# TinyMPC/tinympc-matlab

Hardware: AMD Instinct MI355X
Metric: ADMM iterations/s, batched quadrotor nx=12 nu=4 N=50 (instance-iterations/s, whole job) (higher is better)
Workload: dtype f64

## Files before the change

__graft_entry__.py:

```python
from __future__ import annotations

import hashlib
import importlib.util
import os
import shutil
import subprocess
import sys

ROOT = os.path.dirname(os.path.abspath(__file__))
if ROOT not in sys.path:
    sys.path.insert(0, ROOT)
PKG_DIR = os.path.join(ROOT, "tinympc-matlab_amd")
PKG_NAME = "tinympc_matlab_amd"
CSRC = os.path.join(PKG_DIR, "csrc")
HIP_LIB = os.path.join(PKG_DIR, "libtinympc_hip.so")
ORACLE_DIR = os.path.join(ROOT, "oracle")
REFERENCE_SRC = "/root/reference/src/codegen_src"

HIP_SOURCES = ["tinympc_kernels.hip", "tinympc_precompute_rows.hip", "tinympc_solve.hip", "tinympc_solve_b.hip", "tinympc_solve_fam.hip", "tinympc_solve_adapt.hip", "tinympc_solve_c.hip", "tinympc_solve_d.hip", "tinympc_solve_dr.hip", "tinympc_solve_dw.hip", "tinympc_solve_dx.hip", "tinympc_jit.hip", "tinympc_solve_m.hip", "tinympc_precompute_large.hip", "tinympc_handle.hip", "tinympc_plan.hip", "tinympc_session.hip", "tinympc_capi.hip",
               "tinympc_codegen.hip"]
HIP_LINTED = ["tinympc_precompute_rows.hip", "tinympc_solve.hip", "tinympc_solve_b.hip", "tinympc_solve_fam.hip", "tinympc_solve_adapt.hip",
              "tinympc_solve_c.hip", "tinympc_solve_d.hip", "tinympc_solve_dr.hip", "tinympc_solve_dw.hip", "tinympc_solve_dx.hip"]
JIT_EMBEDDED = ["tinympc_device.h", "tinympc_sweep.h", "tinympc_fam_red.h", "tinympc_solve_d_chain.h", "tinympc_solve_dw_chain.h", "tinympc_solve_dx_chain.h",
                "tinympc_solve_e_common.h", "tinympc_solve_dwide.h", "tinympc_solve_d.hip", "tinympc_solve_dw.hip", "tinympc_solve_dx.hip", "tinympc_solve_e.hip",
                "tinympc_solve_f.hip"]
_ROCKET = ["-DTINY_JIT_NX=6", "-DTINY_JIT_NU=3", "-DTINY_JIT_N=100", "-DTINY_JIT_CT=0", "-DTINY_JIT_FAM=1"]
_ROCKET_FAM = ["-DTINY_JIT_E_NROUND=1", "-DTINY_JIT_E_NCONE=2", "-DTINY_JIT_E_CONES={0,0,2},{0,6,8}", "-DTINY_JIT_E_NLX=1", "-DTINY_JIT_E_NLU=0"]
HIP_BUILTINS = [
    ("k_builtin_e_rocket100", "tinympc_solve_e.hip",
     _ROCKET + ["-DTINY_JIT_E_WPG=8", "-DTINY_JIT_E_WPS=2", "-DTINY_JIT_E_S=13"] + _ROCKET_FAM +
     ["-DTINY_JIT_E_GC_LDS=0", "-DTINY_JIT_E_GL_LDS=0", "-DTINY_JIT_E_LX_LDS=0", "-DTINY_JIT_E_KFAM=1", "-DTINY_JIT_E_DREG=1"]),
    ("k_builtin_f_rocket100", "tinympc_solve_f.hip", _ROCKET + ["-DTINY_JIT_F_WPG=4", "-DTINY_JIT_F_S=7"] + _ROCKET_FAM + ["-DTINY_JIT_F_KFAM=1"]),
    ("k_builtin_f_rocket100_session", "tinympc_solve_f.hip", _ROCKET + ["-DTINY_JIT_F_WPG=4", "-DTINY_JIT_F_S=7"] + _ROCKET_FAM + ["-DTINY_JIT_F_KFAM=1", "-DTINY_JIT_F_SESSION=1"]),
]
_NO_FAM = ["-DTINY_JIT_E_NROUND=0", "-DTINY_JIT_E_NCONE=0", "-DTINY_JIT_E_CONES={-1,0,0}", "-DTINY_JIT_E_NLX=0", "-DTINY_JIT_E_NLU=0"]
for _name, _nx, _nu, _N, _wpg, _S in (("cartpole20", 4, 1, 20, 2, 3), ("quadrotor50", 12, 4, 50, 4, 4)):
    for _suffix, _ct, _extra in (("", 1, []), ("_var", 0, []), ("_session", 0, ["-DTINY_JIT_F_SESSION=1"])):
        HIP_BUILTINS.append(("k_builtin_f_%s%s" % (_name, _suffix), "tinympc_solve_f.hip",
                             ["-DTINY_JIT_NX=%d" % _nx, "-DTINY_JIT_NU=%d" % _nu, "-DTINY_JIT_N=%d" % _N, "-DTINY_JIT_CT=%d" % _ct, "-DTINY_JIT_FAM=0",
                              "-DTINY_JIT_F_WPG=%d" % _wpg, "-DTINY_JIT_F_S=%d" % _S] + _NO_FAM + _extra))
BUILD_DIR = os.path.join(ROOT, "build", "hip")
HIP_CFLAGS = ["--offload-arch=gfx950", "-O3", "-std=c++17", "-fPIC", "-fno-gpu-rdc",
              "-Wall", "-Wno-unused-function", "-I" + os.path.join(ROOT, "include"), "-I" + CSRC, "-I" + BUILD_DIR]
HIP_LDFLAGS = ["--offload-arch=gfx950", "-shared", "-fPIC", "-fno-gpu-rdc", "-lhiprtc"]

# ... 296 lines not shown
```

tinympc-matlab_amd/csrc/tinympc_device.h:

```cpp
#pragma once
#ifndef __HIPCC_RTC__
#include <hip/hip_runtime.h>
#endif

namespace tinympc {

__host__ __device__ inline size_t ops_doubles(int W, int KT) { return (size_t)2 * W * KT + 3 * W; }

__host__ __device__ inline size_t table_rows(int N) { return (size_t)N + 2; }

constexpr int V_PAD = 4;
__host__ __device__ inline size_t v_rows(int N) { return (size_t)N + 1 + 2 * V_PAD; }
__host__ __device__ inline size_t tables_doubles(int W, int N) { return 3 * table_rows(N) * W + W; }

#if defined(__HIPCC__) || defined(__HIPCC_RTC__)
__device__ __forceinline__ void host_store(double *p, double v) { __hip_atomic_store(p, v, __ATOMIC_RELAXED, __HIP_MEMORY_SCOPE_SYSTEM); }
#endif

struct PrecomputeParams {
    int nx, nu;
    double rho;
    const double *A, *B, *fdyn, *Qd, *Rd;
    double *Kinf, *Pinf, *Quu_inv, *AmBKt, *APf, *BPf;
    int *info;
// ... 237 lines not shown
    double *rho_inst;
    int batch;
    double rho;
    double *mail;
};
hipError_t launch_setup_init(const SetupInitParams &p, hipStream_t stream);
hipError_t launch_fill_bounds(double *xmin, double *xmax, size_t X, double *umin, double *umax, size_t U, double inf, hipStream_t stream);
hipError_t launch_reset_stats(int *istats, double *dstats, double *rho_inst, int batch, double rho, hipStream_t stream);
size_t lqr_scratch_doubles(int nx, int nu);
size_t precompute_large_scratch_doubles(int nx, int nu);
hipError_t launch_precompute_large(const PrecomputeParams &p, hipStream_t stream);
hipError_t launch_build_operators(const OperatorParams &p, hipStream_t stream);
hipError_t launch_build_tables(const TableParams &p, hipStream_t stream);
hipError_t launch_store_inst_refs(const InstRefStoreParams &p, hipStream_t stream);
hipError_t launch_build_inst_tables(const InstTableParams &p, hipStream_t stream);
enum class SolveExt { Box, Families, Adaptive, InstRefs, InstBounds };
hipError_t launch_solve_a(const SolveParams &p, SolveExt ext, int W, int KT, size_t lds_bytes, hipStream_t stream);
hipError_t launch_solve_b(const SolveParams &p, int W, int KT, size_t lds_bytes, hipStream_t stream);
size_t solve_b_lds_bytes(int nx, int nu, int N, int W);
constexpr int WAVES_PER_GROUP_B = 4;
bool solve_d_supported(int nx, int nu, int N, bool const_tables);
hipError_t launch_solve_d(const SolveParams &p, hipStream_t stream);
hipError_t launch_solve_d_refill(const SolveParams &p, hipStream_t stream);
int solve_d_workgroups(int nu, int N, bool const_tables, int groups);
size_t solve_d_lds_bytes(int nu, int N, bool const_tables);
int solve_d_resident_workgroups(int wpg);
int solve_d_wavefronts_per_workgroup(int nu, int N, bool const_tables);
bool solve_dw_supported(int nx, int nu, int N, bool const_tables);
hipError_t launch_solve_dw(const SolveParams &p, hipStream_t stream);
int solve_dw_workgroups(int nu, int N, int groups);
size_t solve_dw_lds_bytes(int nu, int N);
bool solve_dx_supported(int nx, int nu, int N, bool const_tables);
hipError_t launch_solve_dx(const SolveParams &p, hipStream_t stream);
int solve_dx_workgroups(int nu, int N, int groups);
size_t solve_dx_lds_bytes(int nu, int N);
hipError_t launch_solve_c(const SolveParams &p, int W, int KT, size_t lds_bytes, hipStream_t stream);
hipError_t launch_build_chunk_tables(const ChunkTableParams &p, hipStream_t stream);
size_t f_input_table_doubles(int nu, int S);
hipError_t launch_build_f_input_tables(const ChunkTableParams &p, hipStream_t stream);
void chunk_plan(int N, int *S, int *C, int *Lc);
size_t solve_c_lds_bytes(int nx, int Lc);
size_t solve_c_lds_bytes_refs(int nx, int nu, int N, int Lc);
size_t chunk_table_doubles(int nx, int Lc);
int chunk_ks(int nx);
hipError_t launch_build_adapt(const AdaptTableParams &p, hipStream_t stream);
inline hipError_t ensure_dynamic_lds(const void *fn, size_t bytes, size_t (&cache)[16]) {
// ... 39 lines not shown
```

tinympc-matlab_amd/csrc/tinympc_plan.hip:

```cpp
#include <cstring>
#include "tinympc_handle.h"

using namespace tinympc;
using namespace tinympc::host;

namespace {

void arm_completion_flag(tinympc_solver *s, SolveParams &p) {
    if (!p.host_sol) return;
    s->session_seq += 1;
    p.host_seq = (double)s->session_seq;
    s->flag_pending = true;
}

void decide_layout_d_variants(tinympc_solver *s) {
    if (!s->layout_d) return;
    if (s->d_varying < 0 && !s->tables_const()) {
        if (s->W == 16 && !s->d_jit && solve_d_supported(s->nx, s->nu, s->N, false)) {
            s->d_varying = 1;
        } else {
            s->d_varying_jit = solve_jit_supported(s->W, s->nx, s->nu, s->N, false);
            s->d_varying = s->d_varying_jit ? 1 : 0;
        }
    }
// ... 185 lines not shown
}

static bool refill_applies(const tinympc_solver *s, const LaunchPlan &pl) {
    const bool jit = pl.kernel == KernelId::D_JIT;
    if ((pl.kernel != KernelId::D_COMPILED && !jit) || s->W != 16 || pl.adaptive || pl.families || pl.inst_refs || s->zero_copy_tick || s->st.max_iter <= 0 ||
        s->st.check_termination <= 0)
        return false;
    const char *env = getenv("TINYMPC_REFILL");
    const int mode = env ? atoi(env) : -1;
    if (mode == 0) return false;
    const bool ct = s->tables_const();
    long resident;
    if (jit) resident = solve_jit_resident_wavefronts(s->W, s->nx, s->nu, s->N, ct);
    else {
        const int wpg = solve_d_wavefronts_per_workgroup(s->nu, s->N, ct);
        resident = (long)solve_d_resident_workgroups(wpg) * wpg;
    }
    const bool reachable = s->st.abs_pri_tol > 0.0 && s->st.abs_dua_tol > 0.0;
    if ((long)s->groups <= resident) return false;
    if (!reachable && mode != 1) return false;
    return !jit || solve_jit_refill_supported(s->W, s->nx, s->nu, s->N, ct);
}

int launch(tinympc_solver *s, bool timed) {
    int rc;
    s->flag_pending = false;
    if ((rc = resolve_plan(s))) return rc;
    const LaunchPlan pl = current_plan(s);
    const bool fam = pl.families, adaptive = pl.adaptive;
    if (s->inst_tables() && !pl.inst_refs) {
        const bool r = s->inst.refs(), b = s->inst.bounds;
        return fail(TINYMPC_ERR_UNSUPPORTED, "%s%s%s are not supported %s; %s%s%s", r ? "per-instance references (set_x_ref_batch / set_u_ref_batch)" : "",
                    r && b ? " and " : "", b ? "per-instance bounds (set_bound_constraints_batch)" : "",
                    s->layout_m ? "for systems with nx+nu > 64" : fam ? "with cone / linear constraint families" : "with adaptive rho",
                    r ? "tinympc_set_x_ref / tinympc_set_u_ref return to shared references" : "", r && b ? ", " : "",
                    b ? "tinympc_set_bound_constraints returns to shared bounds" : "");
    }
    if (s->refs_on_host && adaptive) {
        if ((rc = flush_host_refs(s))) return rc;
    }
    if ((rc = refresh_derived(s))) return rc;
    if (adaptive && fam)
        return fail(TINYMPC_ERR_UNSUPPORTED, "adaptive_rho together with cone / linear constraint families is not supported");
    if (s->layout_m && adaptive)
        return fail(TINYMPC_ERR_UNSUPPORTED, "adaptive_rho is not supported for systems with nx+nu > 64");
    if (fam && pl.kernel != KernelId::E && pl.kernel != KernelId::F && pl.kernel != KernelId::M && family_structure(s).beyond_generic())
// ... 63 lines not shown
    }
    p.rho_min = s->st.adaptive_rho_min; p.rho_max = s->st.adaptive_rho_max; p.rho_clip = s->st.adaptive_rho_enable_clipping;
    const bool kernel_takes_cold = (pl.kernel == KernelId::D_COMPILED || pl.kernel == KernelId::D_JIT) && s->st.max_iter > 0;
    if (s->cold_state && !kernel_takes_cold && (rc = materialize_cold_state(s))) return rc;
    p.cold = s->cold_state ? 1 : 0;
    s->cold_state = false;
    if (s->st.max_iter > 0) s->sol_zero_pending = false;
    else if ((rc = materialize_zero_solution(s))) return rc;
    if (refill_applies(s, pl) && !p.x0_mirror && !p.u0_host && !p.host_sol) {
        if (!s->drefill && (rc = dalloc(s, &s->drefill, 1))) return rc;
        HIP_TRY(hipMemsetAsync(s->drefill, 0, sizeof(int), s->stream));
        p.refill_next = s->drefill;
    }
    if (timed) HIP_TRY(hipEventRecord(s->ev0, s->stream));
    switch (pl.kernel) {
        case KernelId::M:
            p.ctab = s->dctab;
            HIP_TRY(launch_solve_m(p, s->stream));
            break;
        case KernelId::D_JIT:
            HIP_TRY(launch_solve_jit(p, s->W, s->stream));
            break;
        case KernelId::D_COMPILED:
            HIP_TRY(s->W == 64 ? launch_solve_dx(p, s->stream) : s->W == 32 ? launch_solve_dw(p, s->stream) : launch_solve_d(p, s->stream));
            break;
        case KernelId::E:
            p.ctab = s->dctab_e; p.chunk_len = s->e_chunk_len; p.chunk_count = s->e_wpg; p.chunk_levels = 1;
            HIP_TRY(launch_solve_e(p, s->fs, s->stream));
            break;
        case KernelId::F:
            p.ctab = s->dctab_f; p.ftab = s->dftab; p.chunk_len = s->f_chunk_len; p.chunk_count = s->f_chunks; p.chunk_levels = 4;
            arm_completion_flag(s, p);
            HIP_TRY(launch_solve_f(p, s->f_fs, s->stream));
            break;
        case KernelId::C:
            p.ctab = s->dctab; p.chunk_len = s->chunk_len; p.chunk_count = s->chunk_count; p.chunk_levels = s->chunk_levels;
            arm_completion_flag(s, p);
            HIP_TRY(launch_solve_c(p, s->W, s->KT, s->lds_bytes_c, s->stream));
            break;
        case KernelId::B:
            HIP_TRY(launch_solve_b(p, s->W, s->KT, s->lds_bytes, s->stream));
            break;
        case KernelId::A:
        case KernelId::FAM_A:
        case KernelId::ADAPT_A: {
            const SolveExt ext = pl.kernel == KernelId::FAM_A ? SolveExt::Families : pl.kernel == KernelId::ADAPT_A ? SolveExt::Adaptive
                                 : pl.inst_bounds ? SolveExt::InstBounds : pl.inst_refs ? SolveExt::InstRefs : SolveExt::Box;
// ... 33 lines not shown
    if (rc) return rc;
    if ((rc = bind_device(s))) return rc;
    s->specialise_asked = true;
    if ((rc = resolve_plan(s))) return rc;
    (void)refill_applies(s, current_plan(s));
    return TINYMPC_OK;
}

int tinympc_get_jit_info(tinympc_solver *s, char *buf, int len) {
    int rc = check_handle(s);
    if (rc) return rc;
    if (!buf || len < 1) return fail(TINYMPC_ERR_INVALID_INPUT, "get_jit_info: buffer required");
    buf[0] = '\0';
    const LaunchPlan pl = current_plan(s);
    const bool ct = s->tables_const();
    if (pl.inst_refs) {
        const char *words = !pl.inst_bounds ? " per-instance-refs" : s->inst.refs() ? " per-instance-refs per-instance-bounds" : " per-instance-bounds";
        if (pl.kernel == KernelId::D_JIT) {
            if ((rc = bind_device(s))) return rc;
            solve_jit_describe(s->W, s->nx, s->nu, s->N, true, false, false, buf, (size_t)len, true);
            strncat(buf, words, (size_t)len - strlen(buf) - 1);
            strncat(buf, " goal", (size_t)len - strlen(buf) - 1);
        } else {
            snprintf(buf, (size_t)len, "compiled-in layout=%c%s%s", pl.layout, words, pl.kernel == KernelId::D_COMPILED ? " goal" : "");
        }
        return TINYMPC_OK;
    }
    if (!pl.adaptive && !s->f_sig.empty() && !s->f_ok && pl.kernel != KernelId::E && pl.kernel != KernelId::D_JIT && pl.kernel != KernelId::D_COMPILED)
        solve_f_describe(s->nx, s->nu, s->N, ct, pl.families, s->f_fs, buf, (size_t)len);
    else if (!pl.adaptive && !s->e_sig.empty() && !s->e_ok && pl.kernel != KernelId::F && pl.kernel != KernelId::D_JIT && pl.kernel != KernelId::D_COMPILED)
        solve_e_describe(s->nx, s->nu, s->N, ct, pl.families, s->fs, buf, (size_t)len);
    else if (pl.kernel == KernelId::F) solve_f_describe(s->nx, s->nu, s->N, ct, pl.families, s->f_fs, buf, (size_t)len);
    else if (pl.kernel == KernelId::E) solve_e_describe(s->nx, s->nu, s->N, ct, pl.families, s->fs, buf, (size_t)len);
    else if (pl.kernel == KernelId::D_JIT || (s->d_jit_asked && !s->layout_d && !s->layout_m)) {
        if ((rc = bind_device(s))) return rc;
        solve_jit_describe(s->W, s->nx, s->nu, s->N, ct, pl.families && !pl.adaptive, pl.adaptive && !pl.families, buf, (size_t)len);
        if (pl.kernel == KernelId::D_JIT && refill_applies(s, pl)) strncat(buf, " slot-refill", (size_t)len - strlen(buf) - 1);
    } else snprintf(buf, (size_t)len, "compiled-in layout=%c%s", pl.layout, refill_applies(s, pl) ? " slot-refill" : "");
    return TINYMPC_OK;
}

}
```

tinympc-matlab_amd/csrc/tinympc_solve_d.hip:

```cpp
#ifndef TINY_JIT
#include <atomic>
#endif
#include <type_traits>

#include "tinympc_device.h"
#include "tinympc_sweep.h"

#ifndef TINY_REFILL
#if defined(TINY_JIT_REFILL) && TINY_JIT_REFILL
#define TINY_REFILL 1
#else
#define TINY_REFILL 0
#endif
#endif

#define TINY_STR2(x) #x
#define TINY_STR(x) TINY_STR2(x)
namespace tinympc {
template <int NX, int NU>
struct DStep;
}

#ifdef TINY_JIT
#define D_NX TINY_JIT_NX
#define D_NU TINY_JIT_NU
#include "tinympc_solve_d_chain.h"
#else
#define D_NX 12
#define D_NU 4
#include "tinympc_solve_d_chain.h"
#define D_NX 4
#define D_NU 1
#include "tinympc_solve_d_chain.h"
#endif

namespace tinympc {
// ... 342 lines not shown
            static_for<0, 16>([&](auto K) {
                constexpr int o = (K.value < NXU ? K.value : 0) * 16;
                m[K.value] = fma(delta, src[o + (sAd - sOps)], src[o]);
            });
        } else {
            static_for<0, 16>([&](auto K) { m[K.value] = src[(K.value < NXU ? K.value : 0) * 16]; });
        }
    };
    auto vget = [&](auto S) -> double {
        if constexpr (decltype(S)::value >= VL) return Vr[decltype(S)::value - VL];
        else return sVl[decltype(S)::value * 64];
    };

#ifdef TINY_CLOCK_STAMP
    const unsigned long long ck_t0 = __builtin_amdgcn_s_memtime(), ck_r0 = __builtin_amdgcn_s_memrealtime();
#endif
#ifdef TINY_D_PAD
    asm volatile(".rept " TINY_STR(TINY_D_PAD) "\n\ts_nop 0\n\t.endr" ::: "memory");
#endif
#ifdef TINY_D_LOOP_ALIGN
    asm volatile(".p2align " TINY_STR(TINY_D_LOOP_ALIGN) ::: "memory");
#endif
    const int max_iter = p.max_iter;
    for (int it = 0; max_iter > 0; ++it) {
        const int it0 = __builtin_amdgcn_readfirstlane(it);
#if TINY_REFILL
        const bool final_round = REFILL ? false : it0 >= max_iter;
#else
        const bool final_round = it0 >= max_iter;
#endif
        if constexpr (TWO_PER_SIMD) fair_share_priority<NS>(it0, simd_slot);
#if TINY_REFILL
        const bool fin = REFILL ? it_done >= max_iter : final_round;
        const bool wb = pending || (fin && active);
#else
        const bool wb = pending || (final_round && active);
#endif
        if (TINY_RARE(__ballot(wb) != 0ull)) {
            int lane_o = lane;
            asm volatile("" : "+v"(lane_o));
            const int r_o = lane_o & 15, j_o = lane_o >> 4;
            const bool x_o = r_o < NX;
#if TINY_REFILL
            int cur_o = cur;
            if constexpr (REFILL) asm volatile("" : "+v"(cur_o));
            const size_t grp_w = REFILL ? (size_t)(cur_o >> 2) : (size_t)grp;
            const int lane_w = REFILL ? (cur_o & 3) * 16 + r_o : lane_o;
#endif
            if (wb && r_o < NXU) {
// ... 91 lines not shown
                        if (take) {
                            static_for<0, VL>([&](auto S) { sVl[S.value * 64] = 0.0; });
                            if (!x_o && r_o < NXU)
                                for (int i = 0; i < NS; ++i) sDw[i * DS] = 0.0;
                        }
                    } else if (take) {
                        const double *const nG = p.G + grp_n * (N + 1) * 64 + lane_n;
                        const double *const nV = p.V + (grp_n * v_rows(N) + V_PAD) * 64 + lane_n;
                        static_for<0, NS>([&](auto S) { G[S.value] = nG[(S.value + koff) * 64]; });
                        static_for<0, NVR>([&](auto S) { Vr[S.value] = nV[(VL + S.value + koff) * 64]; });
                        static_for<0, VL>([&](auto S) { sVl[S.value * 64] = nV[(S.value + koff) * 64]; });
                        G0 = nG[0];
                        V0 = nV[0];
                        if (!x_o && r_o < NXU) {
                            const double *const nD = p.D + grp_n * (NS * DS) + (nxt & 3) * NU + (r_o - NX);
                            for (int i = 0; i < NS; ++i) sDw[i * DS] = nD[i * DS];
                        }
                    }
#endif
                }
            }
            pending = false;
        }
        if (final_round || __ballot(active) == 0ull) break;
        const int it1 = it0 + 1;
#if TINY_REFILL
        bool chk = true, check_r = false;
        if constexpr (REFILL) {
            chk = active && (ct > 0) && (((it_done + 1) % ct) == 0);
            check_r = __ballot(chk) != 0ull;
        }
#define TINY_CHECK_PLAIN (__builtin_amdgcn_readfirstlane((int)((ct > 0) && ((it1 % ct) == 0))) != 0)
        const bool check = REFILL ? check_r : TINY_CHECK_PLAIN;
#undef TINY_CHECK_PLAIN
#else
        const bool check = __builtin_amdgcn_readfirstlane((int)((ct > 0) && ((it1 % ct) == 0))) != 0;
#endif

        double pri = 0.0, dua = 0.0;
        bool may = check;
        double m[16];
        load_ops(sMf, m);
        const bool adapt = ADAPT && __builtin_amdgcn_readfirstlane((int)((it0 > 0) && (it0 % 5 == 0))) != 0;
        double a_pr = 0.0, a_pn = 0.0, a_dr = 0.0, a_dn = 0.0;
        double gprev = 0.0;
        double mtr[16];
        if constexpr (ADAPT) {
            if (adapt) static_for<0, 16>([&](auto K) { mtr[K.value] = K.value < NXU ? sAd[2 * 256 + K.value * 16 + r] : 0.0; });
        }
// ... 9 lines not shown
#if TINY_REFILL
                may = __builtin_amdgcn_readfirstlane((int)wave_may_converge_d(__ballot(bad), __ballot(REFILL ? chk : active))) != 0;
#else
                may = __builtin_amdgcn_readfirstlane((int)wave_may_converge_d(__ballot(bad), __ballot(active))) != 0;
#endif
            }
#if TINY_REFILL
            if (TINY_RARE(may) && is_x && active) gV1u[REFILL ? row_offset(cur) : (unsigned)lane] = V0;
#else
            if (TINY_RARE(may) && is_x && active) gV1u[(unsigned)lane] = V0;
#endif
            V0 = snew;
        }
        if constexpr (FAM) {
            double gcn, gln;
            (void)families(x0v, GC0, GL0, gcn, gln);
            if (is_x) {
                GC0 = gcn;
                GL0 = gln;
            }
        }
        double xcur = x0v;
        double dcur = lds_read_async<0>(aD), vcur = 0.0;
        if constexpr (VL > 0) vcur = lds_read_async<0>(aV);
        double locur = lo_c, hicur = hi_c;
        if constexpr (!CT) {
            locur = lds_read_async<W * 8>(aT);
            hicur = lds_read_async<(TOFF + W) * 8>(aT);
        }
        lds_wait_ops(m);
        auto fstep = [&](auto S) {
            constexpr int q = decltype(S)::value;
            double dn = 0.0, vn = 0.0, lon = lo_c, hin = hi_c;
            if constexpr (q + 1 < NS) dn = lds_read_async<(q + 1) * DS * 8>(aD);
            if constexpr (q + 1 < VL) vn = lds_read_async<(q + 1) * 512>(aV);
            if constexpr (!CT && q + 1 < NS) {
                lon = lds_read_async<(q + 2) * W * 8>(aT);
                hin = lds_read_async<(TOFF + (q + 2) * W) * 8>(aT);
            }
            const double xprev = xcur;
            double snew_q;
            if constexpr (q >= VL) {
                if constexpr (K0 && q == 0) xcur = Step::fwd_reg0(dcur, m, c0, locur, hicur, G[q], Vr[q - VL], pri, dua);
                else xcur = Step::fwd_reg(xcur, dcur, m, cf, locur, hicur, G[q], Vr[q - VL], pri, dua);
                snew_q = Vr[q - VL];
            } else {
                double vnew;
                if constexpr (K0 && q == 0) xcur = Step::fwd_lds0(dcur, m, c0, locur, hicur, G[q], vcur, vnew, pri, dua);
                else xcur = Step::fwd_lds(xcur, dcur, m, cf, locur, hicur, G[q], vcur, vnew, pri, dua);
                lds_write_async<q * 512>(aV, vnew);
                snew_q = vnew;
            }
            if constexpr (ADAPT) {
                if (adapt) {
                    const double gnew = G[q], out = xcur;
                    const double t = group_matvec<W, 16>(mtr, is_x ? gnew : 0.0, 0.0);
                    const double dgx = dgr * (is_x ? xprev : out);
                    const double aty = is_x ? (t - gprev) : (gnew + t);
                    a_dn = fmax(fmax(a_dn, fabs(dgx)), fabs(aty));
                    a_dr = fmax(a_dr, fabs(2.0 * dgx + aty));
                    a_pr = fmax(a_pr, fabs(is_x ? snew_q : (out - snew_q)));
                    a_pn = fmax(fmax(a_pn, fabs(snew_q)), is_x ? 0.0 : fabs(out));
                    gprev = gnew;
                }
// ... 164 lines not shown
                constexpr int s2 = s >= 2 ? s - 2 : 0;
                constexpr int s3 = s >= 3 ? s - 3 : 0;
                double v2n = 0.0;
                if constexpr (s >= 2) v2n = vreq(std::integral_constant<int, s3>{});
                const double lr2 = lr_of(std::integral_constant<int, s2>{});
                const double lrmc2 = is_x ? lr2 + cb : cb;
                double a = acc, an, rn;
                if constexpr (ADAPT) Step::bwd_v(a, px, rcur, m, v2cur, G[s2], rhom_lin, lrmc2, nrho_lin, lr2, an, rn);
                else if constexpr (FOLD) Step::bwd_fold(a, px, rcur, m, v2cur, G[s2], rhom, lrmc_f, an, rn);
                else Step::bwd(a, px, rcur, m, v2cur, G[s2], rhom, lrmc2, nrho, lr2, an, rn);
                lds_write_masked<s * DS * 8>(aD, a, wr_d);
                px = a;
                rcur = rnext;
                rnext = rn;
                acc = an;
                v2cur = v2n;
            });
            {
                double a = acc;
                Step::bwd_last(a, px, rcur, m);
                lds_write_masked<0>(aD, a, wr_d);
            }
        }
    }
    lds_wait();
#ifdef TINY_CLOCK_STAMP
    const unsigned long long ck_t1 = __builtin_amdgcn_s_memtime(), ck_r1 = __builtin_amdgcn_s_memrealtime();
#endif

#if TINY_REFILL
    if constexpr (REFILL) return;
#endif
    if (inst_ok && status == 1 && r < NXU) {
        __builtin_amdgcn_fence(__ATOMIC_RELEASE, "wavefront");
        const int rows = is_x ? N : NS;
        double *const wV = p.V + ((size_t)grp * v_rows(N) + V_PAD) * 64 + lane;
        const double *const wV2 = p.V2 + ((size_t)grp * v_rows(N) + V_PAD) * 64 + lane;
        for (int kn = 0; kn < rows; ++kn) wV[kn * 64] = wV2[kn * 64];
    }

    const double res_px = group_max<W>(is_x ? snap_pri : 0.0), res_pu = group_max<W>(is_u ? snap_pri : 0.0);
    const double rho_res = ADAPT ? snap_rho : rho;
    const double res_dx = group_max<W>(is_x ? snap_dua : 0.0) * rho_res, res_du = group_max<W>(is_u ? snap_dua : 0.0) * rho_res;

#ifdef TINY_CLOCK_STAMP
    if (p.scratch && lane == 0) {
        unsigned long long *ck = reinterpret_cast<unsigned long long *>(p.scratch) + 8 * (size_t)grp;
        ck[0] = ck_t1 - ck_t0;
        ck[1] = ck_r1 - ck_r0;
        ck[2] = ck_barrier - ck_entry;
        ck[3] = ck_r0 - ck_barrier;
        ck[4] = __builtin_amdgcn_s_memrealtime() - ck_r1;
        ck[5] = ck_entry;
        ck[6] = __builtin_amdgcn_s_memrealtime();
        ck[7] = (unsigned long long)__builtin_amdgcn_s_getreg((31 << 11) | 4) | ((unsigned long long)__builtin_amdgcn_s_getreg((3 << 11) | 20) << 32);
    }
#endif
    if (inst_ok && r == 0) {
        if constexpr (ADAPT) p.rho_inst[inst] = rho;
        p.istats[inst * 2 + 0] = it_done;
        p.istats[inst * 2 + 1] = status;
        if (res_valid) {
            p.dstats[inst * 4 + 0] = res_px;
            p.dstats[inst * 4 + 1] = res_dx;
            p.dstats[inst * 4 + 2] = res_pu;
            p.dstats[inst * 4 + 3] = res_du;
        }
    }
}

#ifndef TINY_JIT
#if TINY_REFILL
template <int NX, int NU, int N, bool CT, int WPG, int VL>
__global__ void __launch_bounds__(64 * WPG) __attribute__((amdgpu_waves_per_eu(2, 2))) k_admm_solve_d_refill(const SolveParams p) {
#else
template <int NX, int NU, int N, bool CT, int WPG, int VL, bool HOSTX = false>
__global__ void __launch_bounds__(64 * WPG) __attribute__((amdgpu_waves_per_eu(2, 2))) k_admm_solve_d(const SolveParams p) {
#endif
    extern __shared__ __attribute__((aligned(16))) double smem[];
#if TINY_REFILL
    k_admm_solve_d_body<NX, NU, N, CT, WPG, VL, false, false, true, false, true>(p, smem);
#else
    k_admm_solve_d_body<NX, NU, N, CT, WPG, VL, false, false, true, HOSTX>(p, smem);
#endif
}
#if !TINY_REFILL
template <int NX, int NU, int N, int WPG, int VL>
__global__ void __launch_bounds__(64 * WPG) __attribute__((amdgpu_waves_per_eu(2, 2))) k_admm_solve_d_gbnd(const SolveParams p) {
    extern __shared__ __attribute__((aligned(16))) double smem[];
    k_admm_solve_d_body<NX, NU, N, true, WPG, VL, false, false, true, false, false, true>(p, smem);
}
#endif
#endif
// ... 140 lines not shown
hipError_t launch_solve_d(const SolveParams &p, hipStream_t stream) {
    if (p.refill_next) return launch_solve_d_refill(p, stream);
#define X(NX_, NU_, N_)                                       \
    if (p.nx == NX_ && p.nu == NU_ && p.N == N_)              \
        return p.const_tables ? launch_d_one<NX_, NU_, N_, true>(p, stream) : launch_d_one<NX_, NU_, N_, false>(p, stream);
    TINY_D_SHAPES(X)
#undef X
    return hipErrorInvalidValue;
}

size_t solve_d_lds_bytes(int nu, int N, bool const_tables) {
    const int wpg = d_wpg(nu, N, const_tables);
    return d_lds_bytes(nu, N, const_tables, wpg, d_vl(nu, N, const_tables, wpg));
}

int solve_d_workgroups(int nu, int N, bool const_tables, int groups) {
    const int wpg = d_wpg(nu, N, const_tables);
    return (groups + wpg - 1) / wpg;
}

#endif

#endif

}
```

tinympc-matlab_amd/csrc/tinympc_solve_d_chain.h:

```cpp
#if !defined(D_NX) || !defined(D_NU)
#error "define D_NX and D_NU before including tinympc_solve_d_chain.h"
#endif
#if D_NX < 1 || D_NU < 1 || D_NX + D_NU > 16
#error "layout D: 1 <= nx, 1 <= nu, nx + nu <= 16"
#endif

#ifdef TINY_CHAIN_NOALIGN
#define D_AL ""
#define D_MOV64 "v_mov_b64"
#else
#define D_AL ".p2align 3\n\t"
#ifdef TINY_CHAIN_MOV32
#define D_MOV64 "v_mov_b64"
#else
#define D_MOV64 "v_mov_b64_e64"
#endif
#endif
#if defined(TINY_JIT) || defined(TINY_CHAIN_NOP)
#define D_HAZ "s_nop 1\n\t" D_AL
#else
#define D_HAZ D_AL
#endif
#define D_FM_(src, i) "v_fmac_f64_dpp %[a], " src ", %[m" #i "] row_newbcast:" #i " row_mask:0xf bank_mask:0xf\n\t"
#if 0 < D_NX
// ... 183 lines not shown
#define D_I14 ""
#endif
#if 15 >= D_NX && 15 < D_NX + D_NU
#define D_I15 D_FM_("%[d]", 15)
#else
#define D_I15 ""
#endif
#define D_CHAIN_IN D_I0 D_I1 D_I2 D_I3 D_I4 D_I5 D_I6 D_I7 D_I8 D_I9 D_I10 D_I11 D_I12 D_I13 D_I14 D_I15
#define D_CHAIN D_C0 D_C1 D_C2 D_C3 D_C4 D_C5 D_C6 D_C7 D_C8 D_C9 D_C10 D_C11 D_C12 D_C13 D_C14 D_C15
#define D_MOPS                                                                                                      \
    [m0] "v"(m[0]), [m1] "v"(m[1]), [m2] "v"(m[2]), [m3] "v"(m[3]), [m4] "v"(m[4]), [m5] "v"(m[5]), [m6] "v"(m[6]), \
        [m7] "v"(m[7]), [m8] "v"(m[8]), [m9] "v"(m[9]), [m10] "v"(m[10]), [m11] "v"(m[11]), [m12] "v"(m[12]),       \
        [m13] "v"(m[13]), [m14] "v"(m[14]), [m15] "v"(m[15])

#define D_PROJECT                                  \
    "v_add_f64 %[s], %[a], %[g]\n\t"               \
    "v_max_f64 %[sn], %[lo], %[s]\n\t"             \
    "v_min_f64 %[sn], %[hi], %[sn]\n\t"            \
    "v_add_f64 %[g], %[s], -%[sn]\n\t"             \
    "v_add_f64 %[t], %[a], -%[sn]\n\t"             \
    "v_max_f64 %[pri], %[pri], |%[t]|\n\t"         \
    "v_add_f64 %[t], %[v], -%[sn]\n\t"             \
    "v_max_f64 %[dua], %[dua], |%[t]|\n\t"
#define D_P1 "v_add_f64 %[s], %[ap], %[g]\n\t"
#define D_P2 "v_max_f64 %[sn], %[lo], %[s]\n\t"
#define D_P3 "v_min_f64 %[sn], %[hi], %[sn]\n\t"
#define D_P4 "v_add_f64 %[g], %[s], -%[sn]\n\t"
#define D_P5 "v_add_f64 %[t], %[ap], -%[sn]\n\t"
#define D_P6 "v_max_f64 %[pri], %[pri], |%[t]|\n\t"
#define D_P7 "v_add_f64 %[t], %[v], -%[sn]\n\t"
#define D_P8 "v_max_f64 %[dua], %[dua], |%[t]|\n\t"
#define D_CHAIN_WOVEN D_C0 D_P1 D_C1 D_P2 D_C2 D_P3 D_C3 D_P4 D_C4 D_P5 D_C5 D_P6 D_C6 D_P7 D_C7 D_P8 D_C8 D_C9 D_C10 D_C11 D_C12 D_C13 D_C14 D_C15
#define D_PROJECT_PREV D_P1 D_P2 D_P3 D_P4 D_P5 D_P6 D_P7 D_P8
#define D_T1 "v_add_f64 %[t], %[v2], -%[g2]\n\t"
#define D_T2 "v_fma_f64 %[an], %[rhom], %[t], %[lrmc]\n\t"
#define D_T3 "v_fma_f64 %[rn], %[nrho], %[t], %[lr]\n\t"
#define D_CHAIN_BWD_WOVEN D_C0 D_T1 D_C1 D_C2 D_T2 D_C3 D_T3 D_C4 D_C5 D_C6 D_C7 D_C8 D_C9 D_C10 D_C11 D_C12 D_C13 D_C14 D_C15

namespace tinympc {

template <>
struct DStep<D_NX, D_NU> {
    static __device__ __forceinline__ double fwd_reg(double x, double d, const double (&m)[16], double cf, double lo, double hi,
                                                     double &g, double &v, double &pri, double &dua) {
        double a, s, t, sn;
        asm volatile("v_mov_b64 %[a], %[cf]\n\t" D_HAZ D_CHAIN D_PROJECT "v_mov_b64 %[v], %[sn]\n\t"
// ... 6 lines not shown
                                                     double &g, double v, double &vnew, double &pri, double &dua) {
        double a, s, t;
        asm volatile(D_MOV64 " %[a], %[cf]\n\t" D_HAZ D_CHAIN D_PROJECT
                     : [a] "=&v"(a), [s] "=&v"(s), [t] "=&v"(t), [sn] "=&v"(vnew), [g] "+v"(g), [pri] "+v"(pri), [dua] "+v"(dua)
                     : [x] "v"(x), [d] "v"(d), [cf] "v"(cf), [lo] "v"(lo), [hi] "v"(hi), [v] "v"(v), D_MOPS);
        lds_reads_landed();
        return a;
    }
    static __device__ __forceinline__ double fwd_reg0(double d, const double (&m)[16], double c0, double lo, double hi, double &g, double &v,
                                                      double &pri, double &dua) {
        double a, s, t, sn;
        asm volatile("v_mov_b64 %[a], %[cf]\n\t" D_HAZ D_CHAIN_IN D_PROJECT "v_mov_b64 %[v], %[sn]\n\t"
                     : [a] "=&v"(a), [s] "=&v"(s), [t] "=&v"(t), [sn] "=&v"(sn), [g] "+v"(g), [v] "+v"(v), [pri] "+v"(pri), [dua] "+v"(dua)
                     : [d] "v"(d), [cf] "v"(c0), [lo] "v"(lo), [hi] "v"(hi), D_MOPS);
        lds_reads_landed();
        return a;
    }
    static __device__ __forceinline__ double fwd_lds0(double d, const double (&m)[16], double c0, double lo, double hi, double &g, double v,
                                                      double &vnew, double &pri, double &dua) {
        double a, s, t;
        asm volatile(D_MOV64 " %[a], %[cf]\n\t" D_HAZ D_CHAIN_IN D_PROJECT
                     : [a] "=&v"(a), [s] "=&v"(s), [t] "=&v"(t), [sn] "=&v"(vnew), [g] "+v"(g), [pri] "+v"(pri), [dua] "+v"(dua)
                     : [d] "v"(d), [cf] "v"(c0), [lo] "v"(lo), [hi] "v"(hi), [v] "v"(v), D_MOPS);
        lds_reads_landed();
        return a;
    }
    static __device__ __forceinline__ double fwd_reg_woven(double x, double d, const double (&m)[16], double cf, double ap, double lo, double hi,
                                                           double &g, double &v, double &pri, double &dua) {
        double a, s, t, sn;
        asm volatile(D_MOV64 " %[a], %[cf]\n\t" D_HAZ D_CHAIN_WOVEN D_MOV64 " %[v], %[sn]\n\t"
                     : [a] "=&v"(a), [s] "=&v"(s), [t] "=&v"(t), [sn] "=&v"(sn), [g] "+v"(g), [v] "+v"(v), [pri] "+v"(pri), [dua] "+v"(dua)
                     : [x] "v"(x), [d] "v"(d), [cf] "v"(cf), [ap] "v"(ap), [lo] "v"(lo), [hi] "v"(hi), D_MOPS);
        lds_reads_landed();
        return a;
    }
    static __device__ __forceinline__ void project_prev(double ap, double lo, double hi, double &g, double &v, double &pri, double &dua) {
        double s, t, sn;
        asm volatile(D_PROJECT_PREV "v_mov_b64 %[v], %[sn]"
                     : [s] "=&v"(s), [t] "=&v"(t), [sn] "=&v"(sn), [g] "+v"(g), [v] "+v"(v), [pri] "+v"(pri), [dua] "+v"(dua)
                     : [ap] "v"(ap), [lo] "v"(lo), [hi] "v"(hi));
    }
    static __device__ __forceinline__ double fwd_plain(double x, double d, const double (&m)[16], double c) {
        double a;
        asm volatile("v_mov_b64 %[a], %[c]\n\t"
                     "s_nop 1\n\t" D_AL D_CHAIN
                     : [a] "=&v"(a)
// ... 71 lines not shown
#undef D_C13
#undef D_C14
#undef D_C15
#undef D_CHAIN
#undef D_I0
#undef D_I1
#undef D_I2
#undef D_I3
#undef D_I4
#undef D_I5
#undef D_I6
#undef D_I7
#undef D_I8
#undef D_I9
#undef D_I10
#undef D_I11
#undef D_I12
#undef D_I13
#undef D_I14
#undef D_I15
#undef D_CHAIN_IN
#undef D_MOPS
#undef D_PROJECT
#undef D_P1
#undef D_P2
#undef D_P3
#undef D_P4
#undef D_P5
#undef D_P6
#undef D_P7
#undef D_P8
#undef D_CHAIN_WOVEN
#undef D_PROJECT_PREV
#undef D_T1
#undef D_T2
#undef D_T3
#undef D_CHAIN_BWD_WOVEN
#undef D_NX
#undef D_NU
```

Baseline: 993.4 million.

## Add lean D-kernel variant skipping residual computation on non-check iterations

Adds a compiled-in lean variant of the D solve kernel that splits the ADMM loop into runs of iterations with no termination check and one full iteration at each check point. In the lean iterations the forward projection uses new inline-asm helpers that leave out the primal/dual residual max-reductions and the old-slack read. This removes per-iteration residual arithmetic and LDS reads that are only needed when convergence is checked. The cost is a second copy of the kernel per shape, a more involved loop schedule, and larger code; the host selects it for W=16 compiled kernels when no refill, adaptive or family features are in use.

After: 1.133 billion (median of 6 runs). 14.1% higher.

```diff
diff --git a/__graft_entry__.py b/__graft_entry__.py
--- a/__graft_entry__.py
+++ b/__graft_entry__.py
@@ -17,10 +17,10 @@
 ORACLE_DIR = os.path.join(ROOT, "oracle")
 REFERENCE_SRC = "/root/reference/src/codegen_src"
 
-HIP_SOURCES = ["tinympc_kernels.hip", "tinympc_precompute_rows.hip", "tinympc_solve.hip", "tinympc_solve_b.hip", "tinympc_solve_fam.hip", "tinympc_solve_adapt.hip", "tinympc_solve_c.hip", "tinympc_solve_d.hip", "tinympc_solve_dr.hip", "tinympc_solve_dw.hip", "tinympc_solve_dx.hip", "tinympc_jit.hip", "tinympc_solve_m.hip", "tinympc_precompute_large.hip", "tinympc_handle.hip", "tinympc_plan.hip", "tinympc_session.hip", "tinympc_capi.hip",
+HIP_SOURCES = ["tinympc_kernels.hip", "tinympc_precompute_rows.hip", "tinympc_solve.hip", "tinympc_solve_b.hip", "tinympc_solve_fam.hip", "tinympc_solve_adapt.hip", "tinympc_solve_c.hip", "tinympc_solve_d.hip", "tinympc_solve_dr.hip", "tinympc_lean_d.hip", "tinympc_solve_dw.hip", "tinympc_solve_dx.hip", "tinympc_jit.hip", "tinympc_solve_m.hip", "tinympc_precompute_large.hip", "tinympc_handle.hip", "tinympc_plan.hip", "tinympc_session.hip", "tinympc_capi.hip",
                "tinympc_codegen.hip"]
 HIP_LINTED = ["tinympc_precompute_rows.hip", "tinympc_solve.hip", "tinympc_solve_b.hip", "tinympc_solve_fam.hip", "tinympc_solve_adapt.hip",
-              "tinympc_solve_c.hip", "tinympc_solve_d.hip", "tinympc_solve_dr.hip", "tinympc_solve_dw.hip", "tinympc_solve_dx.hip"]
+              "tinympc_solve_c.hip", "tinympc_solve_d.hip", "tinympc_solve_dr.hip", "tinympc_lean_d.hip", "tinympc_solve_dw.hip", "tinympc_solve_dx.hip"]
 JIT_EMBEDDED = ["tinympc_device.h", "tinympc_sweep.h", "tinympc_fam_red.h", "tinympc_solve_d_chain.h", "tinympc_solve_dw_chain.h", "tinympc_solve_dx_chain.h",
                 "tinympc_solve_e_common.h", "tinympc_solve_dwide.h", "tinympc_solve_d.hip", "tinympc_solve_dw.hip", "tinympc_solve_dx.hip", "tinympc_solve_e.hip",
                 "tinympc_solve_f.hip"]
diff --git a/tinympc-matlab_amd/csrc/tinympc_device.h b/tinympc-matlab_amd/csrc/tinympc_device.h
--- a/tinympc-matlab_amd/csrc/tinympc_device.h
+++ b/tinympc-matlab_amd/csrc/tinympc_device.h
@@ -283,6 +283,7 @@
 bool solve_d_supported(int nx, int nu, int N, bool const_tables);
 hipError_t launch_solve_d(const SolveParams &p, hipStream_t stream);
 hipError_t launch_solve_d_refill(const SolveParams &p, hipStream_t stream);
+hipError_t launch_solve_d_lean(const SolveParams &p, hipStream_t stream);
 int solve_d_workgroups(int nu, int N, bool const_tables, int groups);
 size_t solve_d_lds_bytes(int nu, int N, bool const_tables);
 int solve_d_resident_workgroups(int wpg);
diff --git a/tinympc-matlab_amd/csrc/tinympc_lean_d.hip b/tinympc-matlab_amd/csrc/tinympc_lean_d.hip
--- /dev/null
+++ b/tinympc-matlab_amd/csrc/tinympc_lean_d.hip
@@ -0,0 +1,2 @@
+#define TINY_LEAN 1
+#include "tinympc_solve_d.hip"
diff --git a/tinympc-matlab_amd/csrc/tinympc_plan.hip b/tinympc-matlab_amd/csrc/tinympc_plan.hip
--- a/tinympc-matlab_amd/csrc/tinympc_plan.hip
+++ b/tinympc-matlab_amd/csrc/tinympc_plan.hip
@@ -231,6 +231,18 @@
     return !jit || solve_jit_refill_supported(s->W, s->nx, s->nu, s->N, ct);
 }
 
+static bool lean_applies(const tinympc_solver *s, const LaunchPlan &pl) {
+    if (pl.kernel != KernelId::D_COMPILED || s->W != 16 || pl.adaptive || pl.families || s->zero_copy_tick || s->st.max_iter <= 0)
+        return false;
+    if (refill_applies(s, pl)) return false;
+    const char *env = getenv("TINYMPC_LEAN");
+    const int mode = env ? atoi(env) : -1;
+    if (mode == 0) return false;
+    if (mode == 1) return true;
+    const bool reachable = s->st.abs_pri_tol > 0.0 && s->st.abs_dua_tol > 0.0;
+    return s->st.check_termination != 1 || !reachable;
+}
+
 int launch(tinympc_solver *s, bool timed) {
     int rc;
     s->flag_pending = false;
@@ -340,7 +352,8 @@
             HIP_TRY(launch_solve_jit(p, s->W, s->stream));
             break;
         case KernelId::D_COMPILED:
-            HIP_TRY(s->W == 64 ? launch_solve_dx(p, s->stream) : s->W == 32 ? launch_solve_dw(p, s->stream) : launch_solve_d(p, s->stream));
+            if (lean_applies(s, pl) && !p.x0_mirror && !p.u0_host && !p.refill_next) HIP_TRY(launch_solve_d_lean(p, s->stream));
+            else HIP_TRY(s->W == 64 ? launch_solve_dx(p, s->stream) : s->W == 32 ? launch_solve_dw(p, s->stream) : launch_solve_d(p, s->stream));
             break;
         case KernelId::E:
             p.ctab = s->dctab_e; p.chunk_len = s->e_chunk_len; p.chunk_count = s->e_wpg; p.chunk_levels = 1;
@@ -420,7 +433,8 @@
             strncat(buf, words, (size_t)len - strlen(buf) - 1);
             strncat(buf, " goal", (size_t)len - strlen(buf) - 1);
         } else {
-            snprintf(buf, (size_t)len, "compiled-in layout=%c%s%s", pl.layout, words, pl.kernel == KernelId::D_COMPILED ? " goal" : "");
+            snprintf(buf, (size_t)len, "compiled-in layout=%c%s%s%s", pl.layout, words, pl.kernel == KernelId::D_COMPILED ? " goal" : "",
+                     lean_applies(s, pl) ? " lean" : "");
         }
         return TINYMPC_OK;
     }
@@ -434,8 +448,8 @@
         if ((rc = bind_device(s))) return rc;
         solve_jit_describe(s->W, s->nx, s->nu, s->N, ct, pl.families && !pl.adaptive, pl.adaptive && !pl.families, buf, (size_t)len);
         if (pl.kernel == KernelId::D_JIT && refill_applies(s, pl)) strncat(buf, " slot-refill", (size_t)len - strlen(buf) - 1);
-    } else snprintf(buf, (size_t)len, "compiled-in layout=%c%s", pl.layout, refill_applies(s, pl) ? " slot-refill" : "");
-    return TINYMPC_OK;
-}
-
-}
+    } else snprintf(buf, (size_t)len, "compiled-in layout=%c%s%s", pl.layout, refill_applies(s, pl) ? " slot-refill" : "", lean_applies(s, pl) ? " lean" : "");
+    return TINYMPC_OK;
+}
+
+}
diff --git a/tinympc-matlab_amd/csrc/tinympc_solve_d.hip b/tinympc-matlab_amd/csrc/tinympc_solve_d.hip
--- a/tinympc-matlab_amd/csrc/tinympc_solve_d.hip
+++ b/tinympc-matlab_amd/csrc/tinympc_solve_d.hip
@@ -12,6 +12,13 @@
 #else
 #define TINY_REFILL 0
 #endif
+#endif
+
+#ifndef TINY_LEAN
+#define TINY_LEAN 0
+#endif
+#if TINY_LEAN && (TINY_REFILL || defined(TINY_JIT))
+#error "TINY_LEAN: compiled-in plain kernels only"
 #endif
 
 #define TINY_STR2(x) #x
@@ -400,9 +407,16 @@
     asm volatile(".p2align " TINY_STR(TINY_D_LOOP_ALIGN) ::: "memory");
 #endif
     const int max_iter = p.max_iter;
+#if TINY_LEAN
+    auto iteration = [&](auto LEAN_, const int it) __attribute__((always_inline)) -> bool {
+        constexpr bool LEANI = decltype(LEAN_)::value;
+#else
     for (int it = 0; max_iter > 0; ++it) {
+#endif
         const int it0 = __builtin_amdgcn_readfirstlane(it);
-#if TINY_REFILL
+#if TINY_LEAN
+        const bool final_round = !LEANI && it0 >= max_iter;
+#elif TINY_REFILL
         const bool final_round = REFILL ? false : it0 >= max_iter;
 #else
         const bool final_round = it0 >= max_iter;
@@ -540,9 +554,15 @@
             }
             pending = false;
         }
+#if TINY_LEAN
+        if (final_round || __ballot(active) == 0ull) return true;
+#else
         if (final_round || __ballot(active) == 0ull) break;
+#endif
         const int it1 = it0 + 1;
-#if TINY_REFILL
+#if TINY_LEAN
+        const bool check = !LEANI && __builtin_amdgcn_readfirstlane((int)((ct > 0) && ((it1 % ct) == 0))) != 0;
+#elif TINY_REFILL
         bool chk = true, check_r = false;
         if constexpr (REFILL) {
             chk = active && (ct > 0) && (((it_done + 1) % ct) == 0);
@@ -598,7 +618,11 @@
         }
         double xcur = x0v;
         double dcur = lds_read_async<0>(aD), vcur = 0.0;
+#if TINY_LEAN
+        if constexpr (VL > 0 && !LEANI) vcur = lds_read_async<0>(aV);
+#else
         if constexpr (VL > 0) vcur = lds_read_async<0>(aV);
+#endif
         double locur = lo_c, hicur = hi_c;
         if constexpr (!CT) {
             locur = lds_read_async<W * 8>(aT);
@@ -609,13 +633,32 @@
             constexpr int q = decltype(S)::value;
             double dn = 0.0, vn = 0.0, lon = lo_c, hin = hi_c;
             if constexpr (q + 1 < NS) dn = lds_read_async<(q + 1) * DS * 8>(aD);
+#if TINY_LEAN
+            if constexpr (q + 1 < VL && !LEANI) vn = lds_read_async<(q + 1) * 512>(aV);
+#else
             if constexpr (q + 1 < VL) vn = lds_read_async<(q + 1) * 512>(aV);
+#endif
             if constexpr (!CT && q + 1 < NS) {
                 lon = lds_read_async<(q + 2) * W * 8>(aT);
                 hin = lds_read_async<(TOFF + (q + 2) * W) * 8>(aT);
             }
             const double xprev = xcur;
             double snew_q;
+#if TINY_LEAN
+            if constexpr (LEANI) {
+                if constexpr (q >= VL) {
+                    if constexpr (K0 && q == 0) xcur = Step::fwd_reg0_nores(dcur, m, c0, locur, hicur, G[q], Vr[q - VL]);
+                    else xcur = Step::fwd_reg_nores(xcur, dcur, m, cf, locur, hicur, G[q], Vr[q - VL]);
+                    snew_q = Vr[q - VL];
+                } else {
+                    double vnew;
+                    if constexpr (K0 && q == 0) xcur = Step::fwd_lds0_nores(dcur, m, c0, locur, hicur, G[q], vnew);
+                    else xcur = Step::fwd_lds_nores(xcur, dcur, m, cf, locur, hicur, G[q], vnew);
+                    lds_write_async<q * 512>(aV, vnew);
+                    snew_q = vnew;
+                }
+            } else
+#endif
             if constexpr (q >= VL) {
                 if constexpr (K0 && q == 0) xcur = Step::fwd_reg0(dcur, m, c0, locur, hicur, G[q], Vr[q - VL], pri, dua);
                 else xcur = Step::fwd_reg(xcur, dcur, m, cf, locur, hicur, G[q], Vr[q - VL], pri, dua);
@@ -826,7 +869,29 @@
                 lds_write_masked<0>(aD, a, wr_d);
             }
         }
-    }
+#if TINY_LEAN
+        return false;
+    };
+    const bool reachable = p.abs_pri_tol > 0.0 && p.abs_dua_tol > 0.0;
+    const int last_check = ct > 0 ? (max_iter / ct) * ct : 0;
+    for (int it = 0; max_iter > 0;) {
+        int nres = max_iter + 1;
+        if (ct > 0 && reachable) nres = (it / ct + 1) * ct;
+        else if (last_check > it) nres = last_check;
+        const int lean_end = __builtin_amdgcn_readfirstlane(nres - 1 < max_iter ? nres - 1 : max_iter);
+        bool over = false;
+        for (; it < lean_end; ++it) {
+            if (iteration(std::true_type{}, it)) {
+                over = true;
+                break;
+            }
+        }
+        if (over || iteration(std::false_type{}, it)) break;
+        ++it;
+    }
+#else
+    }
+#endif
     lds_wait();
 #ifdef TINY_CLOCK_STAMP
     const unsigned long long ck_t1 = __builtin_amdgcn_s_memtime(), ck_r1 = __builtin_amdgcn_s_memrealtime();
@@ -873,6 +938,58 @@
     }
 }
 
+#if TINY_LEAN
+template <int NX, int NU, int N, bool CT, int WPG, int VL>
+__global__ void __launch_bounds__(64 * WPG) __attribute__((amdgpu_waves_per_eu(2, 2))) k_admm_solve_d_lean(const SolveParams p) {
+    extern __shared__ __attribute__((aligned(16))) double smem[];
+    k_admm_solve_d_body<NX, NU, N, CT, WPG, VL>(p, smem);
+}
+template <int NX, int NU, int N, int WPG, int VL>
+__global__ void __launch_bounds__(64 * WPG) __attribute__((amdgpu_waves_per_eu(2, 2))) k_admm_solve_d_gbnd_lean(const SolveParams p) {
+    extern __shared__ __attribute__((aligned(16))) double smem[];
+    k_admm_solve_d_body<NX, NU, N, true, WPG, VL, false, false, true, false, false, true>(p, smem);
+}
+
+__host__ __device__ constexpr int d_wpg(int nu, int N, bool ct) { return d_vl(nu, N, ct, 4) >= 0 ? 4 : 8; }
+
+template <int NX, int NU, int N, bool CT>
+static hipError_t launch_d_one(const SolveParams &p, hipStream_t stream) {
+    constexpr int WPG = d_wpg(NU, N, CT);
+    constexpr int VL = d_vl(NU, N, CT, WPG);
+    if constexpr (VL < 0) {
+        return hipErrorInvalidValue;
+    } else {
+        constexpr size_t lds = d_lds_bytes(NU, N, CT, WPG, VL);
+        static size_t lds_set_l[16] = {0}, lds_set_lgoal[16] = {0};
+        const int wgs = (p.groups + WPG - 1) / WPG;
+        if (p.x0_mirror || p.u0_host || p.refill_next) return hipErrorInvalidValue;
+        if (p.iref_pn) {
+            if constexpr (!CT) {
+                return hipErrorInvalidValue;
+            } else {
+                if (!p.iref_lr || !p.ibnd) return hipErrorInvalidValue;
+                auto fn = &k_admm_solve_d_gbnd_lean<NX, NU, N, WPG, VL>;
+                hipError_t e = ensure_dynamic_lds(reinterpret_cast<const void *>(fn), lds, lds_set_lgoal);
+                if (e != hipSuccess) return e;
+                hipLaunchKernelGGL(fn, dim3(wgs), dim3(64 * WPG), lds, stream, p);
+            }
+        } else {
+            auto fn = &k_admm_solve_d_lean<NX, NU, N, CT, WPG, VL>;
+            hipError_t e = ensure_dynamic_lds(reinterpret_cast<const void *>(fn), lds, lds_set_l);
+            if (e != hipSuccess) return e;
+            hipLaunchKernelGGL(fn, dim3(wgs), dim3(64 * WPG), lds, stream, p);
+        }
+        return hipGetLastError();
+    }
+}
+
+hipError_t launch_solve_d_lean(const SolveParams &p, hipStream_t stream) {
+    if (p.nx == 12 && p.nu == 4 && p.N == 50) return p.const_tables ? launch_d_one<12, 4, 50, true>(p, stream) : launch_d_one<12, 4, 50, false>(p, stream);
+    if (p.nx == 4 && p.nu == 1 && p.N == 20) return p.const_tables ? launch_d_one<4, 1, 20, true>(p, stream) : launch_d_one<4, 1, 20, false>(p, stream);
+    if (p.nx == 4 && p.nu == 1 && p.N == 10) return p.const_tables ? launch_d_one<4, 1, 10, true>(p, stream) : launch_d_one<4, 1, 10, false>(p, stream);
+    return hipErrorInvalidValue;
+}
+#else
 #ifndef TINY_JIT
 #if TINY_REFILL
 template <int NX, int NU, int N, bool CT, int WPG, int VL>
@@ -1059,5 +1176,6 @@
 #endif
 
 #endif
-
-}
+#endif
+
+}
diff --git a/tinympc-matlab_amd/csrc/tinympc_solve_d_chain.h b/tinympc-matlab_amd/csrc/tinympc_solve_d_chain.h
--- a/tinympc-matlab_amd/csrc/tinympc_solve_d_chain.h
+++ b/tinympc-matlab_amd/csrc/tinympc_solve_d_chain.h
@@ -229,6 +229,11 @@
     "v_max_f64 %[pri], %[pri], |%[t]|\n\t"         \
     "v_add_f64 %[t], %[v], -%[sn]\n\t"             \
     "v_max_f64 %[dua], %[dua], |%[t]|\n\t"
+#define D_PROJECT_NORES                            \
+    "v_add_f64 %[s], %[a], %[g]\n\t"               \
+    "v_max_f64 %[sn], %[lo], %[s]\n\t"             \
+    "v_min_f64 %[sn], %[hi], %[sn]\n\t"            \
+    "v_add_f64 %[g], %[s], -%[sn]\n\t"
 #define D_P1 "v_add_f64 %[s], %[ap], %[g]\n\t"
 #define D_P2 "v_max_f64 %[sn], %[lo], %[s]\n\t"
 #define D_P3 "v_min_f64 %[sn], %[hi], %[sn]\n\t"
@@ -281,6 +286,40 @@
         asm volatile(D_MOV64 " %[a], %[cf]\n\t" D_HAZ D_CHAIN_IN D_PROJECT
                      : [a] "=&v"(a), [s] "=&v"(s), [t] "=&v"(t), [sn] "=&v"(vnew), [g] "+v"(g), [pri] "+v"(pri), [dua] "+v"(dua)
                      : [d] "v"(d), [cf] "v"(c0), [lo] "v"(lo), [hi] "v"(hi), [v] "v"(v), D_MOPS);
+        lds_reads_landed();
+        return a;
+    }
+    static __device__ __forceinline__ double fwd_reg_nores(double x, double d, const double (&m)[16], double cf, double lo, double hi, double &g,
+                                                           double &v) {
+        double a, s;
+        asm volatile("v_mov_b64 %[a], %[cf]\n\t" D_HAZ D_CHAIN D_PROJECT_NORES
+                     : [a] "=&v"(a), [s] "=&v"(s), [g] "+v"(g), [sn] "+v"(v)
+                     : [x] "v"(x), [d] "v"(d), [cf] "v"(cf), [lo] "v"(lo), [hi] "v"(hi), D_MOPS);
+        lds_reads_landed();
+        return a;
+    }
+    static __device__ __forceinline__ double fwd_lds_nores(double x, double d, const double (&m)[16], double cf, double lo, double hi, double &g,
+                                                           double &vnew) {
+        double a, s;
+        asm volatile(D_MOV64 " %[a], %[cf]\n\t" D_HAZ D_CHAIN D_PROJECT_NORES
+                     : [a] "=&v"(a), [s] "=&v"(s), [g] "+v"(g), [sn] "=&v"(vnew)
+                     : [x] "v"(x), [d] "v"(d), [cf] "v"(cf), [lo] "v"(lo), [hi] "v"(hi), D_MOPS);
+        lds_reads_landed();
+        return a;
+    }
+    static __device__ __forceinline__ double fwd_reg0_nores(double d, const double (&m)[16], double c0, double lo, double hi, double &g, double &v) {
+        double a, s;
+        asm volatile("v_mov_b64 %[a], %[cf]\n\t" D_HAZ D_CHAIN_IN D_PROJECT_NORES
+                     : [a] "=&v"(a), [s] "=&v"(s), [g] "+v"(g), [sn] "+v"(v)
+                     : [d] "v"(d), [cf] "v"(c0), [lo] "v"(lo), [hi] "v"(hi), D_MOPS);
+        lds_reads_landed();
+        return a;
+    }
+    static __device__ __forceinline__ double fwd_lds0_nores(double d, const double (&m)[16], double c0, double lo, double hi, double &g, double &vnew) {
+        double a, s;
+        asm volatile(D_MOV64 " %[a], %[cf]\n\t" D_HAZ D_CHAIN_IN D_PROJECT_NORES
+                     : [a] "=&v"(a), [s] "=&v"(s), [g] "+v"(g), [sn] "=&v"(vnew)
+                     : [d] "v"(d), [cf] "v"(c0), [lo] "v"(lo), [hi] "v"(hi), D_MOPS);
         lds_reads_landed();
         return a;
     }
@@ -398,6 +437,7 @@
 #undef D_CHAIN_IN
 #undef D_MOPS
 #undef D_PROJECT
+#undef D_PROJECT_NORES
 #undef D_P1
 #undef D_P2
 #undef D_P3
```
